# Rintazero/ft8_demodulator

Measured on AMD Instinct MI355X. Metric: 15-s FT8 slots/sec (full decode) + LDPC candidates/sec, 1/2/4/8 MI355X, higher is better.
Workload: dtype f32 (STFT, sync score) / f64 (LLR, BP); 1 GPU; BASELINE config 3: batch of 256 independent 15-s slots per GPU, 12 kHz, K=300 candidates, min_score=2, 20 BP iterations (config 5 shape at N>1); slots_per_gpu=256, max_candidates=300, min_score=2, pipeline_depth=2, parallelism=slot-sharded x1

## Files before the change

ft8_demodulator_amd/csrc/sync.hip:

```cpp
#include <climits>

#include "ft8_internal.h"
#include "heap_replay.h"

namespace ft8 {
namespace {

__constant__ int kCostasD[7] = {3, 1, 4, 0, 6, 5, 2};
constexpr int kCostasC[7] = {3, 1, 4, 0, 6, 5, 2};

constexpr int kScoreThreads = 256;
constexpr size_t kScoreLdsBudget = 64 * 1024;

struct ScoreArgs {
  const void* wf;
  int T, F, sps, bpt, num_blocks;
  int t0, NT, NF;
  int rlo, nrows;
  void* scores;
  uint64_t* smask;
  int nseg;
  RowSummary* rowsum;
  double min_score;
  int cmp_f64;
  int n_slots, n_bands, n_ctiles;
};

template <typename T>
__device__ __forceinline__ bool passes(T s, double ms, int cmp_f64) {
  if (s == (T)-INFINITY) return false;
  if (cmp_f64) return !((double)s < ms);
  return !(s < (T)ms);
}

template <typename T, bool LDS, int TW>
__global__ __launch_bounds__(kScoreThreads) void k_score(ScoreArgs a) {
  FT8_RACE_PROLOGUE();
  extern __shared__ __attribute__((aligned(16))) unsigned char smem[];
  T* tile = reinterpret_cast<T*>(smem);
  const int slot = blockIdx.y;
  const int c0 = blockIdx.x * TW;
  const T* wf = reinterpret_cast<const T*>(a.wf) + (int64_t)slot * a.T * a.F;
  const int ncols = min(TW + 7 * a.bpt, a.F - c0);
  if constexpr (LDS) {
    const int n = a.nrows * ncols;
    for (int i = threadIdx.x; i < n; i += kScoreThreads) {
      const int r = i / ncols, c = i - r * ncols;
      tile[i] = wf[(int64_t)(a.rlo + r) * a.F + c0 + c];
    }
    __syncthreads();
  }
  auto get = [&](int row, int col) -> T {
    if constexpr (LDS) return tile[(row - a.rlo) * ncols + (col - c0)];
    else return wf[(int64_t)row * a.F + col];
  };
  const int lane_col = threadIdx.x % TW;
  const int rgroup = threadIdx.x / TW;
  constexpr int kGroups = kScoreThreads / TW;
  const int af = c0 + lane_col;
  T* out = reinterpret_cast<T*>(a.scores) + (int64_t)slot * a.NT * a.NF;
  RowSummary* rs = a.rowsum + (int64_t)slot * a.NT * a.nseg;
  const int sps = a.sps, bpt = a.bpt, nb = a.num_blocks;
  for (int ti = rgroup; ti < a.NT; ti += kGroups) {
    if (af >= a.NF) continue;
    const int at = a.t0 + ti;
    const int base = floordiv(at, sps);
    T score = (T)0;
    int n = 0;
#pragma unroll
    for (int m = 0; m < 3; ++m) {
#pragma unroll
      for (int k = 0; k < 7; ++k) {
        const int block = 36 * m + k;
        const int ba = base + block;
        if (ba < 0 || ba >= nb) continue;
        const int tone = kCostasD[k];
        const int row = at + block * sps;
        const int col = af + tone * bpt;
        const T p = get(row, col);
        if (tone > 0) { score += (T)(p - get(row, col - bpt)); n++; }
        if (tone < 7) { score += (T)(p - get(row, col + bpt)); n++; }
        if (k > 0 && ba > 0) { score += (T)(p - get(row - sps, col)); n++; }
        if (k < 6 && ba + 1 < nb) { score += (T)(p - get(row + sps, col)); n++; }
      }
    }
    T res;
    if (n == 0 || isnan(score) || isinf(score)) res = (T)-INFINITY;
    else res = score / (T)n;
    out[(int64_t)ti * a.NF + af] = res;
    if (passes(res, a.min_score, a.cmp_f64)) {
      RowSummary* e = rs + (int64_t)ti * a.nseg + af / kSegCols;
      atomicAdd(&e->count, 1u);
      atomicMax(&e->maxkey, order_key((double)res));
      const int c = af % kSegCols;
      atomicOr(reinterpret_cast<unsigned long long*>(
                   &a.smask[(((int64_t)slot * a.NT + ti) * a.nseg + af / kSegCols) * 2 + (c & 1)]),
               1ull << (c >> 1));
    }
  }
}

template <typename T>
__global__ void k_score_list(const T* wf, int Tn, int F, int sps, int bpt, const int32_t* cand, int n, T* out,
                             int32_t* err) {
  const int i = blockIdx.x * blockDim.x + threadIdx.x;
  if (i >= n) return;
  const int at = cand[2 * i], af = cand[2 * i + 1];
  const int nb = Tn / sps;
  bool bad = false;
  auto get = [&](int64_t t, int64_t f) -> T {
    if (f < 0) f += F;
    if (t < 0) t += Tn;
    if (f < 0 || f >= F || t < 0 || t >= Tn) { bad = true; return (T)0; }
    return wf[t * F + f];
  };
  const int base = floordiv(at, sps);
  T score = (T)0;
  int cnt = 0;
  for (int m = 0; m < 3; ++m) {
    for (int k = 0; k < 7; ++k) {
      const int block = 36 * m + k;
      const int ba = base + block;
      if (ba < 0 || ba >= nb) continue;
      const int tone = kCostasD[k];
      const int64_t row = (int64_t)at + (int64_t)block * sps, col = (int64_t)af + (int64_t)tone * bpt;
      const T p = get(row, col);
      if (tone > 0) { score += (T)(p - get(row, col - bpt)); cnt++; }
      if (tone < 7) { score += (T)(p - get(row, col + bpt)); cnt++; }
      if (k > 0 && ba > 0) { score += (T)(p - get(row - sps, col)); cnt++; }
      if (k < 6 && ba + 1 < nb) { score += (T)(p - get(row + sps, col)); cnt++; }
    }
  }
  out[i] = (cnt == 0 || isnan(score) || isinf(score)) ? (T)-INFINITY : score / (T)cnt;
  err[i] = bad ? 1 : 0;
}

constexpr int kS2TW = 128;
constexpr int kS2R = 22;
constexpr int kS2Waves = 8;
constexpr int kS2Rows = (kS2R + kS2Waves - 1) / kS2Waves;
constexpr int kS2Threads = kS2Waves * kWave;
typedef float f32x2 __attribute__((ext_vector_type(2)));

template <int BPT, int SPS>
struct S2Geom {
  static constexpr int P = (kS2TW + 7 * BPT + 3) & ~3;
  static constexpr int H = kS2R + 8;
  static constexpr int kFloats = H * P;
  static constexpr int Q = P / 4;
  static constexpr int kIter = (H * Q + kS2Threads - 1) / kS2Threads;
};

__device__ __forceinline__ int fkey(float v) {
  const int i = __float_as_int(v);
  return i ^ ((i >> 31) & 0x7fffffff);
}
template <int CTRL>
__device__ __forceinline__ int dpp_max(int k) {
  return max(k, __builtin_amdgcn_mov_dpp(k, CTRL, 0xf, 0xf, false));
}
__device__ __forceinline__ float wave_max(float v) {
  int k = fkey(v);
  k = dpp_max<0x128>(k);
  k = dpp_max<0x124>(k);
  k = dpp_max<0x122>(k);
  k = dpp_max<0x121>(k);
  const int m = max(max(__builtin_amdgcn_readlane(k, 0), __builtin_amdgcn_readlane(k, 16)),
                    max(__builtin_amdgcn_readlane(k, 32), __builtin_amdgcn_readlane(k, 48)));
  return __int_as_float(m ^ ((m >> 31) & 0x7fffffff));
}

template <int BPT>
__device__ __forceinline__ f32x2 ld2(const float* p) {
  if constexpr (BPT % 2 == 0) return *(const volatile __attribute__((address_space(3))) f32x2*)p;
  else return f32x2{p[0], p[1]};
}

template <int BPT, int SPS>
struct S2Stage {
  int row0[S2Geom<BPT, SPS>::kIter];
  int off0[S2Geom<BPT, SPS>::kIter];
};
template <int BPT, int SPS>
__device__ __forceinline__ S2Stage<BPT, SPS> s2_stage(int F, int a0, int c0) {
  using G = S2Geom<BPT, SPS>;
  S2Stage<BPT, SPS> st;
#pragma unroll
  for (int it = 0; it < G::kIter; ++it) {
    const int idx = (int)threadIdx.x + it * kS2Threads;
    const int rw = idx / G::Q, q4 = idx - rw * G::Q;
    const int row = a0 - SPS + SPS * rw, col = c0 + 4 * q4;
    const bool ok = idx < G::H * G::Q && col < F;
    st.row0[it] = ok ? row : INT_MIN / 2;
    st.off0[it] = row * F + col;
  }
  return st;
}
template <int BPT, int SPS>
__device__ __forceinline__ void s2_load(const float* wf, int T, int F, const S2Stage<BPT, SPS>& st, int m,
                                        float4 (&v)[S2Geom<BPT, SPS>::kIter]) {
  using G = S2Geom<BPT, SPS>;
  const int drow = 36 * m * SPS;
  const float* wb = wf + (int64_t)drow * F;
#pragma unroll
  for (int it = 0; it < G::kIter; ++it) {
    const int row = st.row0[it] + drow;
    v[it] = make_float4(0.f, 0.f, 0.f, 0.f);
    if ((unsigned)row < (unsigned)T) v[it] = *reinterpret_cast<const float4*>(wb + st.off0[it]);
  }
}

template <int BPT, int SPS, bool COMPACT>
__global__ __launch_bounds__(kS2Threads) void k_score2(ScoreArgs a) {
  FT8_RACE_PROLOGUE();
  static_assert(kS2TW == kSegCols, "a workgroup's columns are one score segment");
  using G = S2Geom<BPT, SPS>;
  constexpr int P = G::P;
  extern __shared__ __attribute__((aligned(16))) unsigned char smem[];
  float* tile = reinterpret_cast<float*>(smem);
  const int id = blockIdx.x;
  const int per = a.n_bands * a.n_ctiles;
  const int q = id >> 3;
  const int slot = (q / per) * 8 + (id & 7);
  if (slot >= a.n_slots) return;
  const int r = q % per;
  const int band = r / a.n_ctiles, ct = r - band * a.n_ctiles;
  const int nbpc = a.n_bands / SPS;
  const int cls = band / nbpc, i0 = (band - cls * nbpc) * kS2R;
  const int cnt = (a.NT - cls + SPS - 1) / SPS;
  if (i0 >= cnt) return;
  const int a0 = a.t0 + cls + SPS * i0;
  const int c0 = ct * kS2TW;
  const float* wf = reinterpret_cast<const float*>(a.wf) + (int64_t)slot * a.T * a.F;
  const bool vec = (a.F & 3) == 0;

  const int w = __builtin_amdgcn_readfirstlane(threadIdx.x >> 6);
  const int lane = threadIdx.x & 63;
  const int af = c0 + 2 * lane;
  const int nb = a.num_blocks;
  const int rows = min(kS2R, cnt - i0);
  f32x2 score[kS2Rows];
  int n[kS2Rows];
#pragma unroll
  for (int u = 0; u < kS2Rows; ++u) {
    score[u] = f32x2{0.0f, 0.0f};
    n[u] = 0;
  }

  float4 v[G::kIter];
  const S2Stage<BPT, SPS> stg = s2_stage<BPT, SPS>(a.F, a0, c0);
  if (vec) s2_load<BPT, SPS>(wf, a.T, a.F, stg, 0, v);
#pragma unroll 1
  for (int m = 0; m < 3; ++m) {
    if (m > 0) __syncthreads();
    if (vec) {
#pragma unroll
      for (int it = 0; it < G::kIter; ++it) {
        const int idx = (int)threadIdx.x + it * kS2Threads;
        if (idx < G::H * G::Q) reinterpret_cast<float4*>(tile)[idx] = v[it];
      }
      if (m < 2) s2_load<BPT, SPS>(wf, a.T, a.F, stg, m + 1, v);
    } else {
      for (int i = threadIdx.x; i < G::kFloats; i += kS2Threads) {
        const int rr = i / P, cc = i - rr * P;
        const int row = a0 + 36 * m * SPS - SPS + SPS * rr, col = c0 + cc;
        float x = 0.0f;
        if (row >= 0 && row < a.T && col < a.F) x = wf[(int64_t)row * a.F + col];
        tile[i] = x;
      }
    }
    __syncthreads();
#pragma unroll
    for (int u = 0; u < kS2Rows; ++u) {
      const int j = w + u * kS2Waves;
      if (j >= rows) continue;
      const int lo = floordiv(a0, SPS) + j + 36 * m;
      const float* tb = tile + j * P + 2 * lane;
      if (lo >= 0 && lo <= nb - 7) {
#pragma unroll
        for (int k = 0; k < 7; ++k) {
          const int tone = kCostasC[k];
          const float* rp = tb + (k + 1) * P + tone * BPT;
          const f32x2 pw = ld2<BPT>(rp);
          if (tone > 0) score[u] += pw - ld2<BPT>(rp - BPT);
          if (tone < 7) score[u] += pw - ld2<BPT>(rp + BPT);
          if (k > 0) score[u] += pw - ld2<BPT>(rp - P);
          if (k < 6) score[u] += pw - ld2<BPT>(rp + P);
        }
        n[u] += 25;
      } else if (lo + 6 >= 0 && lo < nb) {
#pragma unroll
        for (int k = 0; k < 7; ++k) {
          const int ba = lo + k;
          if (ba < 0 || ba >= nb) continue;
          const int tone = kCostasC[k];
          const float* rp = tb + (k + 1) * P + tone * BPT;
          const f32x2 pw = ld2<BPT>(rp);
          if (tone > 0) { score[u] += pw - ld2<BPT>(rp - BPT); n[u]++; }
          if (tone < 7) { score[u] += pw - ld2<BPT>(rp + BPT); n[u]++; }
          if (k > 0 && ba > 0) { score[u] += pw - ld2<BPT>(rp - P); n[u]++; }
          if (k < 6 && ba + 1 < nb) { score[u] += pw - ld2<BPT>(rp + P); n[u]++; }
        }
      }
    }
  }

  float* out = reinterpret_cast<float*>(a.scores) + (COMPACT ? 0 : (int64_t)slot * a.NT * a.NF);
  RowSummary* rs = a.rowsum + (int64_t)slot * a.NT * a.nseg;
#pragma unroll
  for (int u = 0; u < kS2Rows; ++u) {
    const int j = w + u * kS2Waves;
    if (j >= rows) continue;
    float res[2];
#pragma unroll
    for (int c = 0; c < 2; ++c) {
      const float sc = score[u][c];
      res[c] = (n[u] == 0 || isnan(sc) || isinf(sc)) ? -INFINITY : sc / (float)n[u];
    }
    const int ti = a0 + SPS * j - a.t0;
    const bool v0 = af < a.NF, v1 = af + 1 < a.NF;
    const bool p0 = v0 && passes(res[0], a.min_score, a.cmp_f64);
    const bool p1 = v1 && passes(res[1], a.min_score, a.cmp_f64);
    const uint64_t b0 = __ballot(p0), b1 = __ballot(p1);
    const int64_t seg = ((int64_t)slot * a.NT + ti) * a.nseg + ct;
    if (COMPACT) {
      const uint64_t below = (1ull << lane) - 1ull;
      const int r0 = __popcll(b0 & below) + __popcll(b1 & below);
      float* sv = out + seg * kSegCols;
      if (p0) sv[r0] = res[0];
      if (p1) sv[r0 + (p0 ? 1 : 0)] = res[1];
    } else {
      float* orow = out + (int64_t)ti * a.NF;
      if (v0) orow[af] = res[0];
      if (v1) orow[af + 1] = res[1];
    }
    if (lane == 0) *reinterpret_cast<ulonglong2*>(a.smask + 2 * seg) = make_ulonglong2(b0, b1);
    const unsigned cnt = (unsigned)(__popcll(b0) + __popcll(b1));
    unsigned long long key = 0ull;
    if (cnt) {
      float mx = p0 ? res[0] : -INFINITY;
      if (p1) mx = fmaxf(mx, res[1]);
      mx = wave_max(mx);
      key = order_key((double)mx);
    }
    if (lane == 0) {
      RowSummary e;
      e.count = cnt;
      e.pad = 0;
      e.maxkey = key;
      rs[seg - (int64_t)slot * a.NT * a.nseg] = e;
    }
  }
}

template <int BPT, int SPS, bool COMPACT>
hipError_t launch_score2(const SyncLaunch& L, const ScoreArgs& a0, hipStream_t s) {
  using G = S2Geom<BPT, SPS>;
  ScoreArgs a = a0;
  a.n_bands = SPS * ((((L.NT + SPS - 1) / SPS) + kS2R - 1) / kS2R);
  a.n_ctiles = (L.NF + kS2TW - 1) / kS2TW;
  const size_t lds = sizeof(float) * G::kFloats;
  static_assert(sizeof(float) * S2Geom<4, 4>::kFloats <= 64 * 1024, "one band fits the default LDS limit");
  static_assert(sizeof(float) * G::kFloats <= 160 * 1024, "one band fits the CU's LDS");
  const int groups = (L.n_slots + 7) / 8;
  const int64_t blocks = (int64_t)groups * 8 * a.n_bands * a.n_ctiles;
  return lds_launch(k_score2<BPT, SPS, COMPACT>, dim3((unsigned)blocks), dim3(kS2Threads), lds, s, a);
}

bool score2_path(const SyncLaunch& L) {
  return !L.wf_f64 && L.bpt == L.sps && ((L.bpt >= 1 && L.bpt <= 4) || L.bpt == 10);
}
template <int B>
hipError_t launch_score2_any(const SyncLaunch& L, const ScoreArgs& a, hipStream_t s) {
  return score_compact(L) ? launch_score2<B, B, true>(L, a, s) : launch_score2<B, B, false>(L, a, s);
}

template <typename T, int TW>
hipError_t launch_score_t(const SyncLaunch& L, hipStream_t s) {
  ScoreArgs a{};
  a.wf = L.wf;
  a.T = L.T;
  a.F = L.F;
  a.sps = L.sps;
  a.bpt = L.bpt;
  a.num_blocks = L.T / L.sps;
  a.t0 = L.t0;
  a.NT = L.NT;
  a.NF = L.NF;
  a.scores = L.scores;
  a.smask = L.smask;
  a.nseg = n_segments(L.NF);
  a.rowsum = L.rowsum;
  a.min_score = L.min_score;
  a.cmp_f64 = L.min_score_f64;
  a.n_slots = L.n_slots;
  hipError_t e = hipSuccess;
  if constexpr (sizeof(T) == 4) {
    if (score2_path(L)) {
      switch (L.bpt) {
        case 1: return launch_score2_any<1>(L, a, s);
        case 2: return launch_score2_any<2>(L, a, s);
        case 3: return launch_score2_any<3>(L, a, s);
        case 4: return launch_score2_any<4>(L, a, s);
        case 10: return launch_score2_any<10>(L, a, s);
        default: break;
      }
    }
  }
  e = hipMemsetAsync(L.smask, 0, sizeof(uint64_t) * 2 * (size_t)L.n_slots * L.NT * a.nseg, s);
  if (e != hipSuccess) return e;
  e = hipMemsetAsync(L.rowsum, 0, sizeof(RowSummary) * (size_t)L.n_slots * L.NT * a.nseg, s);
  if (e != hipSuccess) return e;
  a.rlo = max(0, L.t0 - L.sps);
  const int rhi = min(L.T - 1, L.t0 + L.NT - 1 + 79 * L.sps);
  a.nrows = rhi - a.rlo + 1;
  const int ncols = TW + 7 * L.bpt;
  const size_t lds = (size_t)a.nrows * ncols * sizeof(T);
  dim3 grid((L.NF + TW - 1) / TW, L.n_slots);
  if (lds <= kScoreLdsBudget)
    hipLaunchKernelGGL((k_score<T, true, TW>), grid, dim3(kScoreThreads), lds, s, a);
  else
    hipLaunchKernelGGL((k_score<T, false, TW>), grid, dim3(kScoreThreads), 0, s, a);
  return hipGetLastError();
}

constexpr int kSelThreads = 1024;
constexpr int kSelWaves = kSelThreads / kWave;

struct SelectArgs {
  const void* scores;
  int64_t total;
  int NF, t0, N;
  double min_score;
  int cmp_f64;
  int32_t* cand;
  double* cand_score;
  int32_t* cand_count;
  int32_t* warn;
  const RowSummary* rowsum;
  int NT;
  int32_t* tie;
  const uint64_t* smask;
  int nseg;
  int compact;
};

__device__ int block_excl_sum(int v, int* sh, int* total) {
  const int lane = threadIdx.x & 63, w = threadIdx.x >> 6;
  int x = v;
#pragma unroll
  for (int o = 1; o < 64; o <<= 1) {
    int y = __shfl_up(x, o);
    if (lane >= o) x += y;
  }
  if (lane == 63) sh[w] = x;
  __syncthreads();
  if (threadIdx.x == 0) {
    int acc = 0;
    for (int i = 0; i < kSelWaves; ++i) { int t = sh[i]; sh[i] = acc; acc += t; }
    sh[kSelWaves] = acc;
  }
  __syncthreads();
  const int r = sh[w] + x - v;
  *total = sh[kSelWaves];
  __syncthreads();
  return r;
}
__device__ void bitonic(double* key, int* sec, int* pay, int n) {
  int m = 1;
  while (m < n) m <<= 1;
  for (int i = n + threadIdx.x; i < m; i += kSelThreads) { key[i] = INFINITY; sec[i] = 0x7fffffff; pay[i] = -1; }
  __syncthreads();
  for (int k = 2; k <= m; k <<= 1) {
    for (int j = k >> 1; j > 0; j >>= 1) {
      for (int i = threadIdx.x; i < m; i += kSelThreads) {
        const int l = i ^ j;
        if (l > i) {
          const bool up = (i & k) == 0;
          const bool gt = key[i] > key[l] || (key[i] == key[l] && sec[i] > sec[l]);
          if (gt == up) {
            double tk = key[i]; key[i] = key[l]; key[l] = tk;
            int ts = sec[i]; sec[i] = sec[l]; sec[l] = ts;
            int tp = pay[i]; pay[i] = pay[l]; pay[l] = tp;
          }
        }
      }
      __syncthreads();
    }
  }
}

__device__ __forceinline__ bool kv_less(double ka, int sa, double kb, int sb) {
  return ka < kb || (ka == kb && sa < sb);
}
__device__ void sort_kv(double* key, int* sec, int* pay, int n) {
  if (n > kSelThreads) {
    bitonic(key, sec, pay, n);
    return;
  }
  int m = 1;
  while (m < n) m <<= 1;
  const int t = threadIdx.x;
  double k_ = INFINITY;
  int s_ = 0x7fffffff, p_ = -1;
  if (t < n) {
    k_ = key[t];
    s_ = sec[t];
    p_ = pay[t];
  }
  for (int k = 2; k <= m; k <<= 1) {
    for (int j = k >> 1; j > 0; j >>= 1) {
      double ko;
      int so, po;
      if (j >= kWave) {
        __syncthreads();
        if (t < m) {
          key[t] = k_;
          sec[t] = s_;
          pay[t] = p_;
        }
        __syncthreads();
        const int q = t ^ j;
        ko = t < m ? key[q] : k_;
        so = t < m ? sec[q] : s_;
        po = t < m ? pay[q] : p_;
      } else {
        ko = __shfl_xor(k_, j);
        so = __shfl_xor(s_, j);
        po = __shfl_xor(p_, j);
      }
      const bool up = (t & k) == 0, lower = (t & j) == 0;
      const bool take = (up == lower) ? kv_less(ko, so, k_, s_) : kv_less(k_, s_, ko, so);
      if (take && t < m) {
        k_ = ko;
        s_ = so;
        p_ = po;
      }
    }
  }
  __syncthreads();
  if (t < n) {
    key[t] = k_;
    sec[t] = s_;
    pay[t] = p_;
  }
  __syncthreads();
}

__device__ unsigned long long block_max_u64(unsigned long long v, unsigned long long* sh) {
  const int lane = threadIdx.x & 63, w = threadIdx.x >> 6;
#pragma unroll
  for (int o = 32; o > 0; o >>= 1) {
    const unsigned long long y = __shfl_xor(v, o);
    v = y > v ? y : v;
  }
  if (lane == 0) sh[w] = v;
  __syncthreads();
  unsigned long long m = 0;
  for (int i = 0; i < kSelWaves; ++i) m = sh[i] > m ? sh[i] : m;
  __syncthreads();
  return m;
}

__device__ __forceinline__ uint64_t spread32(uint32_t v) {
  uint64_t x = v;
  x = (x | (x << 16)) & 0x0000FFFF0000FFFFull;
  x = (x | (x << 8)) & 0x00FF00FF00FF00FFull;
  x = (x | (x << 4)) & 0x0F0F0F0F0F0F0F0Full;
  x = (x | (x << 2)) & 0x3333333333333333ull;
  x = (x | (x << 1)) & 0x5555555555555555ull;
  return x;
}
__device__ __forceinline__ int select_bit(uint64_t w, int k) {
  int pos = 0;
#pragma unroll
  for (int width = 32; width > 0; width >>= 1) {
    const int c = __popcll(w & ((1ull << width) - 1ull));
    if (k >= c) {
      k -= c;
      w >>= width;
      pos += width;
    }
  }
  return pos;
}
__device__ __forceinline__ int seg_rank(uint64_t e, uint64_t o, int col) {
  const int l = col >> 1;
  const uint64_t below = (1ull << l) - 1ull;
  return __popcll(e & ((col & 1) ? (below << 1 | 1ull) : below)) + __popcll(o & below);
}

template <typename T>
__global__ __launch_bounds__(kSelThreads) void k_select(SelectArgs a) {
  FT8_RACE_PROLOGUE();
  __shared__ double s_key[kMaxCandidates + 2];
  __shared__ int s_sec[kMaxCandidates + 2];
  __shared__ int s_pay[kMaxCandidates + 2];
  __shared__ int s_rank[kMaxCandidates];
  __shared__ T s_val[kMaxCandidates];
  __shared__ int s_segoff[kSelThreads];
  __shared__ uint64_t s_cm[kSelThreads][2];
  __shared__ int s_isum[kSelWaves + 1];
  __shared__ unsigned long long s_umax[kSelWaves];
  __shared__ int s_flag[6];
  __shared__ double s_am_v[kSelWaves];
  __shared__ int s_am_i[kSelWaves];

  const int slot = blockIdx.x;
  const int nseg = a.nseg;
  const int64_t seg0 = (int64_t)slot * a.NT * nseg;
  const uint64_t* mk = a.smask + 2 * seg0;
  auto value = [&](int sg, int j, int c) -> T {
    if (a.compact) return reinterpret_cast<const T*>(a.scores)[(seg0 + sg) * kSegCols + j];
    const int row = sg / nseg;
    return reinterpret_cast<const T*>(a.scores)[(int64_t)slot * a.total + (int64_t)row * a.NF + c];
  };
  const RowSummary* rsum = a.rowsum + (int64_t)slot * a.NT * nseg;
  auto row_count_key = [&](int r, int* cnt, unsigned long long* key) {
    int c_ = 0;
    unsigned long long k_ = 0ull;
    const RowSummary* rr = rsum + (int64_t)r * nseg;
    for (int s0 = 0; s0 < nseg; s0 += 16) {
      uint4 e[16];
#pragma unroll
      for (int u = 0; u < 16; ++u)
        e[u] = s0 + u < nseg ? *reinterpret_cast<const uint4*>(rr + s0 + u) : make_uint4(0u, 0u, 0u, 0u);
#pragma unroll
      for (int u = 0; u < 16; ++u) {
        const unsigned long long k2 = ((unsigned long long)e[u].w << 32) | e[u].z;
        c_ += (int)e[u].x;
        k_ = k2 > k_ ? k2 : k_;
      }
    }
    *cnt = c_;
    *key = k_;
  };
  const int N = a.N;

  if (threadIdx.x == 0) { s_flag[4] = a.NT; s_flag[5] = a.NT; }
  int total_pass = 0;
  unsigned long long gkey = 0, key0 = 0;
  for (int r0 = 0; r0 < a.NT; r0 += kSelThreads) {
    const int r = r0 + threadIdx.x;
    int cnt = 0;
    unsigned long long key = 0ull;
    if (r < a.NT) row_count_key(r, &cnt, &key);
    if (r0 == 0) key0 = key;
    int ctot;
    const int ex = total_pass + block_excl_sum(cnt, s_isum, &ctot);
    if (cnt > 0 && ex < N && ex + cnt >= N) s_flag[4] = r + 1;
    const unsigned long long m = block_max_u64(key, s_umax);
    gkey = m > gkey ? m : gkey;
    total_pass += ctot;
  }
  __syncthreads();
  if (gkey != 0)
    for (int r = threadIdx.x; r < a.NT; r += kSelThreads) {
      int c_;
      unsigned long long k_ = key0;
      if (r >= kSelThreads) row_count_key(r, &c_, &k_);
      if (k_ == gkey) atomicMin(&s_flag[5], r);
    }
  __syncthreads();
  const int r_end = s_flag[4];
  const int g_row = s_flag[5];
  const T g_val = (T)key_value(gkey);
  const int nsel = min(total_pass, N);

  const int seg_end = r_end * nseg;
  int carry = 0;
  for (int g0 = 0; g0 < seg_end && carry < nsel; g0 += kSelThreads) {
    const int sg = g0 + (int)threadIdx.x;
    uint64_t e = 0, o = 0;
    if (sg < seg_end) {
      e = mk[2 * sg];
      o = mk[2 * sg + 1];
    }
    int ctot;
    const int off = carry + block_excl_sum(__popcll(e) + __popcll(o), s_isum, &ctot);
    s_segoff[threadIdx.x] = off;
    s_cm[threadIdx.x][0] = spread32((uint32_t)e) | (spread32((uint32_t)o) << 1);
    s_cm[threadIdx.x][1] = spread32((uint32_t)(e >> 32)) | (spread32((uint32_t)(o >> 32)) << 1);
    __syncthreads();
    const int n_here = min(kSelThreads, seg_end - g0);
    for (int r = carry + (int)threadIdx.x; r < min(carry + ctot, nsel); r += kSelThreads) {
      int lo = 0, hi = n_here - 1;
      while (lo < hi) {
        const int mid = (lo + hi + 1) >> 1;
        if (s_segoff[mid] <= r) lo = mid;
        else hi = mid - 1;
      }
      const int j = r - s_segoff[lo];
      const uint64_t w0 = s_cm[lo][0];
      const int n0 = __popcll(w0);
      const int col = j < n0 ? select_bit(w0, j) : 64 + select_bit(s_cm[lo][1], j - n0);
      const int sgl = g0 + lo;
      const int row = sgl / nseg;
      const int c = (sgl - row * nseg) * kSegCols + col;
      s_rank[r] = row * a.NF + c;
      s_val[r] = value(sgl, j, c);
    }
    carry += ctot;
    __syncthreads();
  }

  double m1 = -INFINITY;
  for (int i = threadIdx.x; i < nsel; i += kSelThreads) m1 = fmax(m1, (double)s_val[i]);
  {
    const int lane = threadIdx.x & 63, w = threadIdx.x >> 6;
#pragma unroll
    for (int o = 32; o > 0; o >>= 1) m1 = fmax(m1, __shfl_xor(m1, o));
    if (lane == 0) s_am_v[w] = m1;
    __syncthreads();
    m1 = -INFINITY;
    for (int i = 0; i < kSelWaves; ++i) m1 = fmax(m1, s_am_v[i]);
    __syncthreads();
  }
  const bool has_rec = nsel > 0 && total_pass > N && (double)g_val > m1;
  if (threadIdx.x == 0) { s_flag[0] = 0; s_flag[1] = 0; s_flag[3] = 0; s_am_i[0] = 0x7fffffff; }
  __syncthreads();
  if (has_rec) {
    const int64_t rs0 = (int64_t)g_row * nseg;
    for (int c = threadIdx.x; c < a.NF; c += kSelThreads) {
      const int sg = (int)(rs0 + c / kSegCols), col = c % kSegCols;
      const uint64_t e = mk[2 * sg], o = mk[2 * sg + 1];
      if (!(((col & 1) ? o : e) >> (col >> 1) & 1ull)) continue;
      if ((double)value(sg, seg_rank(e, o, col), c) == (double)g_val) atomicMin(&s_am_i[0], g_row * a.NF + c);
    }
    __syncthreads();
  }
  const int gi = s_am_i[0];

  for (int i = threadIdx.x; i < nsel; i += kSelThreads) {
    const int idx = s_rank[i];
    s_key[i] = -(double)s_val[i];
    s_sec[i] = idx;
    s_pay[i] = idx;
  }
  __syncthreads();
  if (has_rec) {
    int top = 0x7fffffff;
    double tk = INFINITY;
    for (int i = threadIdx.x; i < nsel; i += kSelThreads)
      if (s_key[i] < tk || (s_key[i] == tk && s_sec[i] < s_sec[top])) { tk = s_key[i]; top = i; }
    {
      const int lane = threadIdx.x & 63, w = threadIdx.x >> 6;
#pragma unroll
      for (int o = 32; o > 0; o >>= 1) {
        const double ok = __shfl_xor(tk, o);
        const int ot = __shfl_xor(top, o);
        const bool better = ot != 0x7fffffff &&
                            (top == 0x7fffffff || ok < tk || (ok == tk && s_sec[ot] < s_sec[top]));
        if (better) { tk = ok; top = ot; }
      }
      if (lane == 0) { s_am_v[w] = tk; s_isum[w] = top; }
      __syncthreads();
      if (threadIdx.x == 0) {
        for (int i = 1; i < kSelWaves; ++i) {
          const int ot = s_isum[i];
          if (ot == 0x7fffffff) continue;
          if (top == 0x7fffffff || s_am_v[i] < tk || (s_am_v[i] == tk && s_sec[ot] < s_sec[top])) {
            tk = s_am_v[i];
            top = ot;
          }
        }
        s_isum[0] = top;
        s_am_v[0] = tk;
      }
      __syncthreads();
      top = s_isum[0];
      tk = s_am_v[0];
    }
    for (int i = threadIdx.x; i < nsel; i += kSelThreads)
      if (i != top && s_key[i] == tk) s_flag[0] = 1;
    __syncthreads();
    if (threadIdx.x == 0) {
      s_key[top] = -(double)g_val;
      s_sec[top] = gi;
      s_pay[top] = gi;
    }
  }
  __syncthreads();

  sort_kv(s_key, s_sec, s_pay, nsel);
  for (int i = threadIdx.x; i + 1 < nsel; i += kSelThreads)
    if (s_key[i] == s_key[i + 1]) s_flag[0] = 1;
  __syncthreads();

  bool deferred = false;
  if (s_flag[0]) {
    if constexpr (std::is_same<T, float>::value) {
      deferred = a.tie != nullptr && nsel <= kReplayMax;
      if (deferred) {
        int32_t* t = a.tie + (int64_t)slot * tie_stride(a.N);
        for (int i = threadIdx.x; i < nsel; i += kSelThreads) {
          t[i] = s_rank[i];
          t[a.N + i] = s_pay[i];
          t[7 * a.N + 2 + i] = __float_as_int(s_val[i]);
        }
        if (threadIdx.x == 0) {
          t[7 * a.N] = has_rec ? gi : -1;
          t[7 * a.N + 1] = __float_as_int(g_val);
        }
      }
    }
    if (!deferred) {
      for (int i = threadIdx.x; i < nsel; i += kSelThreads) {
        s_key[i] = -(double)s_val[i];
        s_sec[i] = s_rank[i];
      }
      __syncthreads();
      if (threadIdx.x < kWave) {
        const int lane = threadIdx.x;
        int tie = 0;
        {
          for (int n = 1; n < nsel; ++n) {
            const double nk = s_key[n];
            const int ni = s_sec[n];
            const int d = 31 - __clz(n + 1);
            double ak = 0.0;
            int ai = 0;
            if (lane < d) {
              const int pj = ((n + 1) >> (lane + 1)) - 1;
              ak = s_key[pj];
              ai = s_sec[pj];
            }
            const bool lt = lane < d && (nk < ak || (nk == ak && ni < ai));
            const int m = __ffsll((long long)~__ballot(lt)) - 1;
            if (__any(lane < d && lane <= m && nk == ak)) tie = 1;
            if (lane < m) {
              const int dest = lane == 0 ? n : ((n + 1) >> lane) - 1;
              s_key[dest] = ak;
              s_sec[dest] = ai;
            }
            if (lane == 0) {
              const int dest = m == 0 ? n : ((n + 1) >> m) - 1;
              s_key[dest] = nk;
              s_sec[dest] = ni;
            }
            asm volatile("" ::: "memory");
          }
          if (lane == 0 && has_rec) {
            int c = 1;
            while (c < nsel) {
              const int r = c + 1;
              if (r < nsel) {
                if (s_key[c] == s_key[r]) tie = 1;
                const bool cl = s_key[c] < s_key[r] || (s_key[c] == s_key[r] && s_sec[c] < s_sec[r]);
                if (!cl) c = r;
              }
              c = 2 * c + 1;
            }
            s_key[0] = -(double)g_val;
            s_sec[0] = gi;
          }
        }
        if (lane == 0) s_flag[3] = tie;
      }
      __syncthreads();
      for (int i = threadIdx.x; i < nsel; i += kSelThreads) { s_pay[i] = s_sec[i]; s_sec[i] = i; }
      __syncthreads();
      sort_kv(s_key, s_sec, s_pay, nsel);
    }
  }
  if (threadIdx.x == 0) {
    a.cand_count[slot] = nsel;
    a.warn[slot] = (s_flag[3] ? 1 : 0) | (s_flag[0] ? 4 : 0) | (deferred ? 8 : 0);
  }
  for (int i = threadIdx.x; i < nsel; i += kSelThreads) {
    const int idx = s_pay[i];
    a.cand[((int64_t)slot * a.N + i) * 2 + 0] = a.t0 + idx / a.NF;
    a.cand[((int64_t)slot * a.N + i) * 2 + 1] = idx % a.NF;
    a.cand_score[(int64_t)slot * a.N + i] = -s_key[i];
  }
}

constexpr int kTkBits = 11;
constexpr int kTkU = 8;
constexpr int kTkBins = 1 << kTkBits;

template <typename T> struct TkKey;
template <> struct TkKey<float> {
  using K = unsigned;
  static constexpr int kBits = 32;
  __device__ static K of(float v) {
    const unsigned u = __float_as_uint(v);
    return (u >> 31) ? ~u : (u | 0x80000000u);
  }
};
template <> struct TkKey<double> {
  using K = unsigned long long;
  static constexpr int kBits = 64;
  __device__ static K of(double v) { return order_key(v); }
};

template <typename T>
__global__ __launch_bounds__(kSelThreads) void k_topk(SelectArgs a) {
  FT8_RACE_PROLOGUE();
  using K = typename TkKey<T>::K;
  __shared__ double s_key[kMaxCandidates + 2];
  __shared__ int s_sec[kMaxCandidates + 2];
  __shared__ int s_pay[kMaxCandidates + 2];
  __shared__ unsigned s_hist[kTkBins];
  __shared__ int s_isum[kSelWaves + 1];
  __shared__ K s_prefix, s_mask;
  __shared__ int s_need, s_done, s_eqcnt, s_cnt;

  const int slot = blockIdx.x;
  const T* sc = reinterpret_cast<const T*>(a.scores) + (int64_t)slot * a.total;
  const int N = a.N;
  const int total = (int)a.total;
  auto key = [&](int i) -> K {
    const T v = sc[i];
    return passes(v, a.min_score, a.cmp_f64) ? TkKey<T>::of(v) : (K)0;
  };
  if (threadIdx.x == 0) { s_prefix = 0; s_mask = 0; s_need = N; s_done = 0; s_eqcnt = 0; }
  __syncthreads();
  int total_pass = 0;
  for (int pass = 0;; ++pass) {
    int shift = TkKey<T>::kBits - kTkBits * (pass + 1), width = kTkBits;
    if (shift < 0) { width += shift; shift = 0; }
    const K dmask = ((K)1 << width) - 1;
    const K prefix = s_prefix, mask = s_mask;
    for (int b = threadIdx.x; b < kTkBins; b += kSelThreads) s_hist[b] = 0;
    __syncthreads();
    for (int i0 = threadIdx.x; i0 < total; i0 += kTkU * kSelThreads) {
      K kk[kTkU];
#pragma unroll
      for (int u = 0; u < kTkU; ++u) kk[u] = i0 + u * kSelThreads < total ? key(i0 + u * kSelThreads) : (K)0;
#pragma unroll
      for (int u = 0; u < kTkU; ++u)
        if (kk[u] != 0 && (kk[u] & mask) == prefix) atomicAdd(&s_hist[(unsigned)((kk[u] >> shift) & dmask)], 1u);
    }
    __syncthreads();
    const int g = kSelThreads - 1 - (int)threadIdx.x;
    const int hi_c = (int)s_hist[2 * g + 1], lo_c = (int)s_hist[2 * g];
    int in_prefix;
    const int above = block_excl_sum(hi_c + lo_c, s_isum, &in_prefix);
    if (pass == 0) total_pass = in_prefix;
    const int need = s_need;
    if (pass == 0 && total_pass <= N) break;
    if (above < need && need <= above + hi_c + lo_c) {
      const bool top = need <= above + hi_c;
      const int b = top ? 2 * g + 1 : 2 * g;
      const int bc = top ? hi_c : lo_c;
      const int rem = need - (top ? above : above + hi_c);
      s_prefix = prefix | ((K)b << shift);
      s_mask = mask | (dmask << shift);
      s_need = rem;
      s_eqcnt = bc;
      s_done = (bc == rem || shift == 0) ? 1 : 0;
    }
    __syncthreads();
    if (s_done) break;
  }
  const bool take_all = total_pass <= N;
  const K prefix = s_prefix, mask = s_mask;
  const int need_eq = s_need;
  const int nsel = take_all ? total_pass : N;
  int nsort = nsel;
  if (take_all || (N - need_eq) + s_eqcnt <= kMaxCandidates) {
    nsort = take_all ? total_pass : (N - need_eq) + s_eqcnt;
    if (threadIdx.x == 0) s_cnt = 0;
    __syncthreads();
    for (int i0 = threadIdx.x; i0 < total; i0 += kTkU * kSelThreads) {
      K kk[kTkU];
#pragma unroll
      for (int u = 0; u < kTkU; ++u) kk[u] = i0 + u * kSelThreads < total ? key(i0 + u * kSelThreads) : (K)0;
#pragma unroll
      for (int u = 0; u < kTkU; ++u) {
        if (kk[u] != 0 && (take_all || (kk[u] & mask) >= prefix)) {
          const int i = i0 + u * kSelThreads;
          const int pos = atomicAdd(&s_cnt, 1);
          s_key[pos] = -(double)sc[i];
          s_sec[pos] = i;
          s_pay[pos] = i;
        }
      }
    }
  } else {
    const int per = (total + kSelThreads - 1) / kSelThreads;
    const int i_lo = min(total, (int)threadIdx.x * per), i_hi = min(total, i_lo + per);
    int n_above = 0, n_eq = 0;
    for (int i = i_lo; i < i_hi; ++i) {
      const K k = key(i);
      if (k == 0) continue;
      if ((k & mask) > prefix) n_above++;
      else if ((k & mask) == prefix) n_eq++;
    }
    int tot_above, tot_eq;
    int pa = block_excl_sum(n_above, s_isum, &tot_above);
    int pe = block_excl_sum(n_eq, s_isum, &tot_eq);
    for (int i = i_lo; i < i_hi; ++i) {
      const K k = key(i);
      if (k == 0) continue;
      int pos = -1;
      if ((k & mask) > prefix) pos = pa++;
      else if ((k & mask) == prefix) {
        if (pe < need_eq) pos = tot_above + pe;
        pe++;
      }
      if (pos >= 0) {
        s_key[pos] = -(double)sc[i];
        s_sec[pos] = i;
        s_pay[pos] = i;
      }
    }
  }
  __syncthreads();
  sort_kv(s_key, s_sec, s_pay, nsort);
  if (threadIdx.x == 0) {
    a.cand_count[slot] = nsel;
    a.warn[slot] = 0;
  }
  for (int i = threadIdx.x; i < nsel; i += kSelThreads) {
    const int idx = s_pay[i];
    a.cand[((int64_t)slot * a.N + i) * 2 + 0] = a.t0 + idx / a.NF;
    a.cand[((int64_t)slot * a.N + i) * 2 + 1] = idx % a.NF;
    a.cand_score[(int64_t)slot * a.N + i] = -s_key[i];
  }
}


constexpr int kTkcMaxSeg = 8192;
constexpr int kTkcRun = 16;

__device__ __forceinline__ unsigned tk_key(float v) { return TkKey<float>::of(v); }

__device__ __forceinline__ int tkc_seg(const int* off, int nsegs, int d) {
  int lo = 0, hi = nsegs - 1;
  while (lo < hi) {
    const int mid = (lo + hi + 1) >> 1;
    if (off[mid] <= d) lo = mid;
    else hi = mid - 1;
  }
  return lo;
}

__global__ __launch_bounds__(kSelThreads) void k_topkc(SelectArgs a, int M, int V) {
  FT8_RACE_PROLOGUE();
  extern __shared__ __attribute__((aligned(16))) unsigned char smem[];
  const int nsegs = a.NT * a.nseg;
  unsigned* s_hist = reinterpret_cast<unsigned*>(smem);
  int* s_off = reinterpret_cast<int*>(smem + kTkBins * sizeof(unsigned));
  double* s_key = reinterpret_cast<double*>(s_off + ((nsegs + 2) & ~1));
  int* s_sec = reinterpret_cast<int*>(s_key + M);
  int* s_pay = s_sec + M;
  float* s_val = reinterpret_cast<float*>(s_pay + M);
  __shared__ int s_isum[kSelWaves + 1];
  __shared__ unsigned s_prefix, s_mask;
  __shared__ int s_need, s_done, s_eqcnt, s_cnt;

  const int tid = threadIdx.x, lane = tid & (kWave - 1), w = tid >> 6;
  const int slot = blockIdx.x;
  const int64_t seg0 = (int64_t)slot * nsegs;
  const uint64_t* mk = a.smask + 2 * seg0;
  const float* sv = reinterpret_cast<const float*>(a.scores) + seg0 * kSegCols;
  const int N = a.N;

  int carry = 0;
  for (int g0 = 0; g0 < nsegs; g0 += kSelThreads) {
    const int sg = g0 + tid;
    int c = 0;
    if (sg < nsegs) c = __popcll(mk[2 * sg]) + __popcll(mk[2 * sg + 1]);
    int ctot;
    const int ex = block_excl_sum(c, s_isum, &ctot);
    if (sg < nsegs) {
      const int off = carry + ex;
      s_off[sg] = off;
      if (off + c <= V) {
        const float* src = sv + (int64_t)sg * kSegCols;
        for (int j0 = 0; j0 < c; j0 += kTkcRun) {
          float v[kTkcRun];
#pragma unroll
          for (int u = 0; u < kTkcRun; ++u) v[u] = j0 + u < c ? src[j0 + u] : 0.0f;
#pragma unroll
          for (int u = 0; u < kTkcRun; ++u)
            if (j0 + u < c) s_val[off + j0 + u] = v[u];
        }
      }
    }
    carry += ctot;
  }
  const int total = carry;
  if (tid == 0) {
    s_off[nsegs] = total;
    s_prefix = 0;
    s_mask = 0;
    s_need = N;
    s_done = 0;
    s_eqcnt = 0;
    s_cnt = 0;
  }
  __syncthreads();
  const bool staged = total <= V;
  auto visit = [&](auto&& fn) {
    if (staged) {
      for (int d = tid; d < total; d += kSelThreads) fn(d, s_val[d]);
    } else {
      for (int sg = w; sg < nsegs; sg += kSelWaves) {
        const int c0 = s_off[sg], c = s_off[sg + 1] - c0;
        for (int j = lane; j < c; j += kWave) fn(c0 + j, sv[(int64_t)sg * kSegCols + j]);
      }
    }
  };

  const bool take_all = total <= N;
  if (!take_all) {
    for (int pass = 0;; ++pass) {
      int shift = 32 - kTkBits * (pass + 1), width = kTkBits;
      if (shift < 0) { width += shift; shift = 0; }
      const unsigned dmask = (1u << width) - 1u;
      const unsigned prefix = s_prefix, mask = s_mask;
      for (int b = tid; b < kTkBins; b += kSelThreads) s_hist[b] = 0;
      __syncthreads();
      visit([&](int, float v) {
        const unsigned k = tk_key(v);
        if ((k & mask) == prefix) atomicAdd(&s_hist[(k >> shift) & dmask], 1u);
      });
      __syncthreads();
      const int g = kSelThreads - 1 - tid;
      const int hi_c = (int)s_hist[2 * g + 1], lo_c = (int)s_hist[2 * g];
      int in_prefix;
      const int above = block_excl_sum(hi_c + lo_c, s_isum, &in_prefix);
      const int need = s_need;
      if (above < need && need <= above + hi_c + lo_c) {
        const bool top = need <= above + hi_c;
        const int b = top ? 2 * g + 1 : 2 * g;
        const int bc = top ? hi_c : lo_c;
        const int rem = need - (top ? above : above + hi_c);
        s_prefix = prefix | ((unsigned)b << shift);
        s_mask = mask | (dmask << shift);
        s_need = rem;
        s_eqcnt = bc;
        s_done = (bc == rem || shift == 0) ? 1 : 0;
      }
      __syncthreads();
      if (s_done) break;
    }
  }
  const unsigned prefix = s_prefix, mask = s_mask;
  const int need_eq = s_need;
  const int nsel = take_all ? total : N;
  int nsort = take_all ? total : (N - need_eq) + s_eqcnt;
  int m2 = 1;
  while (m2 < nsort) m2 <<= 1;
  if (m2 <= M) {
    visit([&](int d, float v) {
      if (take_all || (tk_key(v) & mask) >= prefix) {
        const int pos = atomicAdd(&s_cnt, 1);
        s_key[pos] = -(double)v;
        s_sec[pos] = d;
        s_pay[pos] = d;
      }
    });
  } else {
    nsort = N;
    const int per = (total + kSelThreads - 1) / kSelThreads;
    const int d_lo = min(total, tid * per), d_hi = min(total, d_lo + per);
    const int sg_lo = d_lo < d_hi ? tkc_seg(s_off, nsegs, d_lo) : 0;
    auto walk = [&](auto&& fn) {
      int sg = sg_lo;
      for (int d = d_lo; d < d_hi; ++d) {
        float v;
        if (staged) {
          v = s_val[d];
        } else {
          while (s_off[sg + 1] <= d) ++sg;
          v = sv[(int64_t)sg * kSegCols + (d - s_off[sg])];
        }
        fn(d, v);
      }
    };
    int n_above = 0, n_eq = 0;
    walk([&](int, float v) {
      const unsigned k = tk_key(v) & mask;
      n_above += k > prefix ? 1 : 0;
      n_eq += k == prefix ? 1 : 0;
    });
    int tot_above, tot_eq;
    int pa = block_excl_sum(n_above, s_isum, &tot_above);
    int pe = block_excl_sum(n_eq, s_isum, &tot_eq);
    walk([&](int d, float v) {
      const unsigned k = tk_key(v) & mask;
      const bool ab = k > prefix, eq = k == prefix;
      const int pos = ab ? pa : (eq && pe < need_eq ? tot_above + pe : -1);
      pa += ab ? 1 : 0;
      pe += eq ? 1 : 0;
      if (pos >= 0) {
        s_key[pos] = -(double)v;
        s_sec[pos] = d;
        s_pay[pos] = d;
      }
    });
  }
  __syncthreads();
  if (tid == 0) {
    a.cand_count[slot] = nsel;
    a.warn[slot] = 0;
  }
  sort_kv(s_key, s_sec, s_pay, nsort);
  for (int i = tid; i < nsel; i += kSelThreads) {
    const int t_ = i;
    const int d = s_pay[i];
    const int sg = tkc_seg(s_off, nsegs, d);
    const int j = d - s_off[sg];
    const uint64_t e = mk[2 * sg], o = mk[2 * sg + 1];
    const uint64_t c0 = spread32((uint32_t)e) | (spread32((uint32_t)o) << 1);
    const int n0 = __popcll(c0);
    const int col = j < n0 ? select_bit(c0, j)
                           : 64 + select_bit(spread32((uint32_t)(e >> 32)) | (spread32((uint32_t)(o >> 32)) << 1), j - n0);
    const int row = sg / a.nseg;
    a.cand[((int64_t)slot * a.N + i) * 2 + 0] = a.t0 + row;
    a.cand[((int64_t)slot * a.N + i) * 2 + 1] = (sg - row * a.nseg) * kSegCols + col;
    a.cand_score[(int64_t)slot * a.N + i] = -s_key[t_];
  }
}

}

bool score_compact(const SyncLaunch& L) {
  return L.compact && score2_path(L) && (!L.topk || (int64_t)L.NT * n_segments(L.NF) <= kTkcMaxSeg);
}

hipError_t launch_score(const SyncLaunch& L, hipStream_t s) {
  if (L.NT <= 0 || L.NF <= 0 || L.n_slots <= 0) return hipSuccess;
  if (L.wf_f64) return launch_score_t<double, 32>(L, s);
  return launch_score_t<float, 64>(L, s);
}

hipError_t launch_score_list(const void* wf, int wf_f64, int T, int F, int sps, int bpt, const int32_t* cand,
                             int n, void* out, int32_t* err, hipStream_t s) {
  if (n <= 0) return hipSuccess;
  const unsigned blocks = (unsigned)((n + 255) / 256);
  if (wf_f64)
    hipLaunchKernelGGL(k_score_list<double>, dim3(blocks), dim3(256), 0, s, (const double*)wf, T, F, sps, bpt, cand,
                       n, (double*)out, err);
  else
    hipLaunchKernelGGL(k_score_list<float>, dim3(blocks), dim3(256), 0, s, (const float*)wf, T, F, sps, bpt, cand, n,
                       (float*)out, err);
  return hipGetLastError();
}

hipError_t launch_select(const SyncLaunch& L, hipStream_t s) {
  if (L.n_slots <= 0) return hipSuccess;
  SelectArgs a{};
  a.scores = L.scores;
  a.total = (int64_t)max(L.NT, 0) * max(L.NF, 0);
  a.NF = max(L.NF, 1);
  a.t0 = L.t0;
  a.N = L.N;
  a.min_score = L.min_score;
  a.cmp_f64 = L.min_score_f64;
  a.cand = L.cand;
  a.cand_score = L.cand_score;
  a.cand_count = L.cand_count;
  a.warn = L.warn;
  a.rowsum = L.rowsum;
  a.tie = L.tie;
  a.NT = max(L.NT, 0);
  a.smask = L.smask;
  a.nseg = n_segments(a.NF);
  a.compact = score_compact(L) ? 1 : 0;
  if (L.topk && a.compact) {
    int M = 64;
    while (M < L.N) M <<= 1;
    const int nsegs = a.NT * a.nseg;
    const size_t fixed = kTkBins * sizeof(unsigned) + (size_t)((nsegs + 2) & ~1) * sizeof(int) +
                         (size_t)M * (sizeof(double) + 2 * sizeof(int));
    const size_t budget = 79 * 1024;
    const int V = (int)std::max<size_t>(4096, fixed < budget ? (budget - fixed) / sizeof(float) : 0);
    const size_t lds = fixed + (size_t)V * sizeof(float);
    return lds_launch(k_topkc, dim3(L.n_slots), dim3(kSelThreads), lds, s, a, M, V);
  }
  if (L.topk) {
    if (L.wf_f64)
      hipLaunchKernelGGL(k_topk<double>, dim3(L.n_slots), dim3(kSelThreads), 0, s, a);
    else
      hipLaunchKernelGGL(k_topk<float>, dim3(L.n_slots), dim3(kSelThreads), 0, s, a);
    return hipGetLastError();
  }
  if (L.wf_f64)
    hipLaunchKernelGGL(k_select<double>, dim3(L.n_slots), dim3(kSelThreads), 0, s, a);
  else
    hipLaunchKernelGGL(k_select<float>, dim3(L.n_slots), dim3(kSelThreads), 0, s, a);
  return hipGetLastError();
}

}
```

Baseline: 139,600 slots/s.

## Move global max search from score kernel into select scan and speed up score epilogue

In the score kernel epilogue, the per-element division is replaced by a reciprocal multiply with an FMA correction for the common counts of 25, 50 and 75. The finite check now uses classf, and the rank computation uses mbcnt instead of popcount masks. The per-row wave_max and order-key computation is skipped in compact mode. The select kernel instead finds the global maximum and its segment by scanning the compact score buffer directly, using prefetched float4 loads and an LDS overflow list, then locates the argmax within a single segment. This removes the reductions from the hot score kernel but adds a full scan of the compact scores to the select kernel, and tie and rounding semantics must match the old path exactly.

```diff
diff --git a/ft8_demodulator_amd/csrc/sync.hip b/ft8_demodulator_amd/csrc/sync.hip
--- a/ft8_demodulator_amd/csrc/sync.hip
+++ b/ft8_demodulator_amd/csrc/sync.hip
@@ -11,6 +11,11 @@
 
 constexpr int kScoreThreads = 256;
 constexpr size_t kScoreLdsBudget = 64 * 1024;
+
+#ifndef FT8_SELECT_SCANS_MAX
+#define FT8_SELECT_SCANS_MAX 1
+#endif
+constexpr bool kSelectScansMax = FT8_SELECT_SCANS_MAX != 0;
 
 struct ScoreArgs {
   const void* wf;
@@ -31,6 +36,15 @@
   if (s == (T)-INFINITY) return false;
   if (cmp_f64) return !((double)s < ms);
   return !(s < (T)ms);
+}
+
+__device__ __forceinline__ float score_threshold(double ms, int cmp_f64) {
+  float f = (float)ms;
+  if (cmp_f64 && (double)f < ms) {
+    const unsigned b = __float_as_uint(f);
+    f = __uint_as_float(f == 0.0f ? 1u : ((b >> 31) ? b - 1u : b + 1u));
+  }
+  return f;
 }
 
 template <typename T, bool LDS, int TW>
@@ -307,28 +321,42 @@
 
   float* out = reinterpret_cast<float*>(a.scores) + (COMPACT ? 0 : (int64_t)slot * a.NT * a.NF);
   RowSummary* rs = a.rowsum + (int64_t)slot * a.NT * a.nseg;
+  const bool v0 = af < a.NF, v1 = af + 1 < a.NF;
+  const float msf = score_threshold(a.min_score, a.cmp_f64);
 #pragma unroll
   for (int u = 0; u < kS2Rows; ++u) {
     const int j = w + u * kS2Waves;
     if (j >= rows) continue;
+    const float nf = (float)n[u];
+    const bool nshort = n[u] == 75 || n[u] == 50 || n[u] == 25;
+    const float rn = n[u] == 75 ? 1.0f / 75.0f : (n[u] == 50 ? 1.0f / 50.0f : 1.0f / 25.0f);
+    const unsigned t0 = (__float_as_uint(score[u][0]) << 1) - 2u, t1 = (__float_as_uint(score[u][1]) << 1) - 2u;
+    const bool tiny = min(t0, t1) < (0x0d800000u << 1) - 2u;
+    f32x2 qt;
+    if (nshort && !__any(tiny)) {
+      const f32x2 r2 = f32x2{rn, rn}, mn2 = f32x2{-nf, -nf};
+      const f32x2 q0 = score[u] * r2;
+      qt = __builtin_elementwise_fma(__builtin_elementwise_fma(mn2, q0, score[u]), r2, q0);
+    } else {
+      qt = f32x2{score[u][0] / nf, score[u][1] / nf};
+    }
+    constexpr int kFinite = 0x1f8;
+    const bool f0 = n[u] != 0 && __builtin_amdgcn_classf(score[u][0], kFinite);
+    const bool f1 = n[u] != 0 && __builtin_amdgcn_classf(score[u][1], kFinite);
     float res[2];
-#pragma unroll
-    for (int c = 0; c < 2; ++c) {
-      const float sc = score[u][c];
-      res[c] = (n[u] == 0 || isnan(sc) || isinf(sc)) ? -INFINITY : sc / (float)n[u];
-    }
+    res[0] = f0 ? qt[0] : -INFINITY;
+    res[1] = f1 ? qt[1] : -INFINITY;
     const int ti = a0 + SPS * j - a.t0;
-    const bool v0 = af < a.NF, v1 = af + 1 < a.NF;
-    const bool p0 = v0 && passes(res[0], a.min_score, a.cmp_f64);
-    const bool p1 = v1 && passes(res[1], a.min_score, a.cmp_f64);
-    const uint64_t b0 = __ballot(p0), b1 = __ballot(p1);
+    const bool p0 = v0 && f0 && !(qt[0] < msf);
+    const bool p1 = v1 && f1 && !(qt[1] < msf);
+    const uint64_t b0 = __builtin_amdgcn_ballot_w64(p0), b1 = __builtin_amdgcn_ballot_w64(p1);
     const int64_t seg = ((int64_t)slot * a.NT + ti) * a.nseg + ct;
     if (COMPACT) {
-      const uint64_t below = (1ull << lane) - 1ull;
-      const int r0 = __popcll(b0 & below) + __popcll(b1 & below);
+      unsigned r0 = __builtin_amdgcn_mbcnt_hi((unsigned)(b0 >> 32), __builtin_amdgcn_mbcnt_lo((unsigned)b0, 0u));
+      r0 = __builtin_amdgcn_mbcnt_hi((unsigned)(b1 >> 32), __builtin_amdgcn_mbcnt_lo((unsigned)b1, r0));
       float* sv = out + seg * kSegCols;
       if (p0) sv[r0] = res[0];
-      if (p1) sv[r0 + (p0 ? 1 : 0)] = res[1];
+      if (p1) sv[r0 + (p0 ? 1u : 0u)] = res[1];
     } else {
       float* orow = out + (int64_t)ti * a.NF;
       if (v0) orow[af] = res[0];
@@ -337,7 +365,7 @@
     if (lane == 0) *reinterpret_cast<ulonglong2*>(a.smask + 2 * seg) = make_ulonglong2(b0, b1);
     const unsigned cnt = (unsigned)(__popcll(b0) + __popcll(b1));
     unsigned long long key = 0ull;
-    if (cnt) {
+    if (!(COMPACT && kSelectScansMax) && cnt) {
       float mx = p0 ? res[0] : -INFINITY;
       if (p1) mx = fmaxf(mx, res[1]);
       mx = wave_max(mx);
@@ -616,20 +644,29 @@
     return reinterpret_cast<const T*>(a.scores)[(int64_t)slot * a.total + (int64_t)row * a.NF + c];
   };
   const RowSummary* rsum = a.rowsum + (int64_t)slot * a.NT * nseg;
-  auto row_count_key = [&](int r, int* cnt, unsigned long long* key) {
+  const bool scan = std::is_same<T, float>::value && kSelectScansMax && a.compact;
+  auto row_count_key = [&](auto counts_only, int r, int* cnt, unsigned long long* key) {
     int c_ = 0;
     unsigned long long k_ = 0ull;
     const RowSummary* rr = rsum + (int64_t)r * nseg;
     for (int s0 = 0; s0 < nseg; s0 += 16) {
-      uint4 e[16];
-#pragma unroll
-      for (int u = 0; u < 16; ++u)
-        e[u] = s0 + u < nseg ? *reinterpret_cast<const uint4*>(rr + s0 + u) : make_uint4(0u, 0u, 0u, 0u);
-#pragma unroll
-      for (int u = 0; u < 16; ++u) {
-        const unsigned long long k2 = ((unsigned long long)e[u].w << 32) | e[u].z;
-        c_ += (int)e[u].x;
-        k_ = k2 > k_ ? k2 : k_;
+      if constexpr (decltype(counts_only)::value) {
+        unsigned e[16];
+#pragma unroll
+        for (int u = 0; u < 16; ++u) e[u] = s0 + u < nseg ? rr[s0 + u].count : 0u;
+#pragma unroll
+        for (int u = 0; u < 16; ++u) c_ += (int)e[u];
+      } else {
+        uint4 e[16];
+#pragma unroll
+        for (int u = 0; u < 16; ++u)
+          e[u] = s0 + u < nseg ? *reinterpret_cast<const uint4*>(rr + s0 + u) : make_uint4(0u, 0u, 0u, 0u);
+#pragma unroll
+        for (int u = 0; u < 16; ++u) {
+          const unsigned long long k2 = ((unsigned long long)e[u].w << 32) | e[u].z;
+          c_ += (int)e[u].x;
+          k_ = k2 > k_ ? k2 : k_;
+        }
       }
     }
     *cnt = c_;
@@ -637,35 +674,127 @@
   };
   const int N = a.N;
 
-  if (threadIdx.x == 0) { s_flag[4] = a.NT; s_flag[5] = a.NT; }
+  constexpr int kPre = 8;
+  constexpr int kScanSegs = kSelThreads / kPre;
+  constexpr int kScanB = 11;
+  const int nsegs = a.NT * nseg;
+  const float* sv = reinterpret_cast<const float*>(a.scores) + seg0 * kSegCols;
+  const int su = threadIdx.x % kPre, sq = threadIdx.x / kPre;
+  int sc_c[kScanB];
+  float4 sc_v[kScanB];
+  auto scan_load = [&](int s0) {
+#pragma unroll
+    for (int k = 0; k < kScanB; ++k) {
+      const int sg = s0 + k * kScanSegs + sq;
+      sc_c[k] = 0;
+      if (sg < nsegs) {
+        sc_c[k] = min((int)rsum[sg].count, kSegCols);
+        sc_v[k] = reinterpret_cast<const float4*>(sv + (int64_t)sg * kSegCols)[su];
+      }
+    }
+  };
+
+  if (threadIdx.x == 0) { s_flag[2] = 0; s_flag[4] = a.NT; s_flag[5] = a.NT; }
   int total_pass = 0;
   unsigned long long gkey = 0, key0 = 0;
-  for (int r0 = 0; r0 < a.NT; r0 += kSelThreads) {
-    const int r = r0 + threadIdx.x;
-    int cnt = 0;
-    unsigned long long key = 0ull;
-    if (r < a.NT) row_count_key(r, &cnt, &key);
-    if (r0 == 0) key0 = key;
-    int ctot;
-    const int ex = total_pass + block_excl_sum(cnt, s_isum, &ctot);
-    if (cnt > 0 && ex < N && ex + cnt >= N) s_flag[4] = r + 1;
-    const unsigned long long m = block_max_u64(key, s_umax);
-    gkey = m > gkey ? m : gkey;
-    total_pass += ctot;
+  auto summaries = [&](auto counts_only) {
+    for (int r0 = 0; r0 < a.NT; r0 += kSelThreads) {
+      const int r = r0 + threadIdx.x;
+      int cnt = 0;
+      unsigned long long key = 0ull;
+      if (r < a.NT) row_count_key(counts_only, r, &cnt, &key);
+      if (r0 == 0) key0 = key;
+      int ctot;
+      const int ex = total_pass + block_excl_sum(cnt, s_isum, &ctot);
+      if (cnt > 0 && ex < N && ex + cnt >= N) s_flag[4] = r + 1;
+      if constexpr (!decltype(counts_only)::value) {
+        const unsigned long long m = block_max_u64(key, s_umax);
+        gkey = m > gkey ? m : gkey;
+      }
+      total_pass += ctot;
+    }
+  };
+  if (scan) {
+    scan_load(0);
+    summaries(std::true_type{});
+  } else {
+    summaries(std::false_type{});
   }
   __syncthreads();
   if (gkey != 0)
     for (int r = threadIdx.x; r < a.NT; r += kSelThreads) {
       int c_;
       unsigned long long k_ = key0;
-      if (r >= kSelThreads) row_count_key(r, &c_, &k_);
+      if (r >= kSelThreads) row_count_key(std::false_type{}, r, &c_, &k_);
       if (k_ == gkey) atomicMin(&s_flag[5], r);
     }
   __syncthreads();
   const int r_end = s_flag[4];
   const int g_row = s_flag[5];
-  const T g_val = (T)key_value(gkey);
+  T g_val = (T)key_value(gkey);
   const int nsel = min(total_pass, N);
+
+  int g_seg = -1;
+  if (scan) {
+    unsigned long long best = 0ull;
+    auto fold = [&](float mx, int sg) {
+      const unsigned b = __float_as_uint(mx + 0.0f);
+      const unsigned k = (b >> 31) ? ~b : (b | 0x80000000u);
+      const unsigned long long x = ((unsigned long long)k << 32) | (unsigned)~sg;
+      best = x > best ? x : best;
+    };
+    auto max4 = [&](float mx, const float4& q, int jj, int c) {
+      mx = (jj + 0 < c && q.x > mx) ? q.x : mx;
+      mx = (jj + 1 < c && q.y > mx) ? q.y : mx;
+      mx = (jj + 2 < c && q.z > mx) ? q.z : mx;
+      mx = (jj + 3 < c && q.w > mx) ? q.w : mx;
+      return mx;
+    };
+    float bmx = -INFINITY;
+    int bsg = -1;
+    for (int s0 = 0; s0 < nsegs; s0 += kScanB * kScanSegs) {
+      if (s0 > 0) scan_load(s0);
+#pragma unroll
+      for (int k = 0; k < kScanB; ++k) {
+        const int sg = s0 + k * kScanSegs + sq;
+        const int c = sc_c[k];
+        if (4 * su < c) {
+          const float mx = max4(-INFINITY, sc_v[k], 4 * su, c);
+          if (mx > bmx) {
+            bmx = mx;
+            bsg = sg;
+          }
+        }
+        if (su == 0 && c > 4 * kPre) {
+          const int at = atomicAdd(&s_flag[2], 1);
+          if (at < kSelThreads) {
+            s_segoff[at] = sg;
+          } else {
+            const float4* src = reinterpret_cast<const float4*>(sv + (int64_t)sg * kSegCols);
+            float mx = -INFINITY;
+            for (int u = kPre; 4 * u < c; ++u) mx = max4(mx, src[u], 4 * u, c);
+            fold(mx, sg);
+          }
+        }
+      }
+    }
+    if (bsg >= 0) fold(bmx, bsg);
+    __syncthreads();
+    const int n_list = min(s_flag[2], kSelThreads);
+    constexpr int kRest = kSegCols / 4 - kPre;
+    for (int i = threadIdx.x; i < n_list * kRest; i += kSelThreads) {
+      const int sg = s_segoff[i / kRest], u = kPre + i % kRest;
+      const int c = min((int)rsum[sg].count, kSegCols);
+      const float4 q = reinterpret_cast<const float4*>(sv + (int64_t)sg * kSegCols)[u];
+      if (4 * u < c) fold(max4(-INFINITY, q, 4 * u, c), sg);
+    }
+    const unsigned long long m = block_max_u64(best, s_umax);
+    if (m != 0ull) {
+      const unsigned k = (unsigned)(m >> 32);
+      g_seg = (int)~(unsigned)m;
+      g_val = (T)__uint_as_float((k >> 31) ? (k & 0x7fffffffu) : ~k);
+    }
+  }
 
   const int seg_end = r_end * nseg;
   int carry = 0;
@@ -719,7 +848,28 @@
   const bool has_rec = nsel > 0 && total_pass > N && (double)g_val > m1;
   if (threadIdx.x == 0) { s_flag[0] = 0; s_flag[1] = 0; s_flag[3] = 0; s_am_i[0] = 0x7fffffff; }
   __syncthreads();
-  if (has_rec) {
+  if (has_rec && g_seg >= 0) {
+    if (threadIdx.x < kWave) {
+      const int lane = threadIdx.x;
+      const float* sp = sv + (int64_t)g_seg * kSegCols;
+      const int c = min((int)rsum[g_seg].count, kSegCols);
+      const float x0 = sp[lane], x1 = sp[lane + kWave];
+      const uint64_t e = mk[2 * g_seg], o = mk[2 * g_seg + 1];
+      const uint64_t h0 = __ballot(lane < c && (T)x0 == g_val), h1 = __ballot(lane + kWave < c && (T)x1 == g_val);
+      const int j = h0 ? __ffsll((long long)h0) - 1 : kWave + __ffsll((long long)h1) - 1;
+      if (lane == (j & (kWave - 1))) {
+        const uint64_t w0 = spread32((uint32_t)e) | (spread32((uint32_t)o) << 1);
+        const int n0 = __popcll(w0);
+        const int col = j < n0 ? select_bit(w0, j)
+                               : 64 + select_bit(spread32((uint32_t)(e >> 32)) | (spread32((uint32_t)(o >> 32)) << 1), j - n0);
+        const int row = g_seg / nseg;
+        s_am_i[0] = row * a.NF + (g_seg - row * nseg) * kSegCols + col;
+        s_am_v[0] = (double)(j < kWave ? x0 : x1);
+      }
+    }
+    __syncthreads();
+    g_val = (T)s_am_v[0];
+  } else if (has_rec) {
     const int64_t rs0 = (int64_t)g_row * nseg;
     for (int c = threadIdx.x; c < a.NF; c += kSelThreads) {
       const int sg = (int)(rs0 + c / kSegCols), col = c % kSegCols;
```

After: 139,600 slots/s (median of 3 runs). No clear change (+0.0%).
